# PierfrancescoArdino/C2M

Hardware: AMD Instinct MI355X
Metric: generator train-step frames/sec at 128x256x7 (higher is better)
Workload: dtype f32; 1 GPU; BASELINE configs[1]: 128x256, 7-frame clips (2 in + 5 predicted), batch 8/GPU, fp32, generator fwd+bwd only (no D), VGG loss on, random-init weights; global_batch=8, parallelism=single

## Files before the change

### c2m_amd/csrc/conv_wino4.hip

```cpp
#include "common.h"
#include "conv_types.h"
#include <stdlib.h>

struct Wino4P {
    const float* U;
    const float* X;
    float* Y;
    const float* bias;
    float* Y2;
    long y2_sn, y2_sc, y2_sh;
    int lo_y, lo_x, ext_y, ext_x;
    int M, K, nimg;
    int Hi, Wi, Ho, Wo;
    int iy0, ix0;
    int reflect;
    long in_sn, out_sn, out_sc, out_sh, out_off;
    int in_sc, in_sh;
    unsigned x_bytes;
    int nchunks, mtiles;
    int act;
    float slope;
    const float* R;
    int r_l;
};

#if !defined(W4_SKEW) && !defined(W4_FUSED)
#define W4_FUSED 1
#endif

constexpr int W4_CK = 8;
constexpr int W4_TH = 4, W4_TW = 8;
constexpr int W4_OR = 4 * W4_TH, W4_OC = 4 * W4_TW;
constexpr int W4_PH = W4_OR + 2, W4_PW = W4_OC + 2;
constexpr int W4_PITCH = 40;
constexpr int W4_PPOS = W4_PH * W4_PITCH;
constexpr int W4_ROWS = (W4_PPOS + 63) / 64;
constexpr int W4_PCS = 722;
constexpr int W4_PBUF = W4_CK * W4_PCS + 48;
constexpr int W4_TAB = W4_ROWS * 64;
constexpr int W4_VBUF = 36 * W4_CK * 32;

#define W4_BT(o0, o1, o2, o3, o4, o5, x0, x1, x2, x3, x4, x5) \
    do {                                                      \
        const float a_ = (x4) - 2.25f * (x2), b_ = 0.75f * (x3) - 1.6875f * (x1);          \
        const float c_ = (x4) - 0.5625f * (x2), e_ = 1.5f * (x3) - 0.84375f * (x1);        \
        o0 = 1.265625f * (x0) - 2.8125f * (x2) + (x4);        \
        o1 = a_ + b_; o2 = a_ - b_; o3 = c_ + e_; o4 = c_ - e_; \
        o5 = 1.265625f * (x1) - 2.8125f * (x3) + (x5);        \
    } while (0)

#ifdef W4_TRACE
__device__ unsigned long long w4_trace_buf[8 * 16 * 4 + 8 * 2];
#define W4_STAMP(i) do { if (blockIdx.x == 0 && lane == 0 && n < 16) sTr[(wave * 16 + n) * 4 + (i)] = clock64(); } while (0)
C2M_API int c2m_wino4_trace_read(unsigned long long* host) {
    return (int)hipMemcpyFromSymbol(host, HIP_SYMBOL(w4_trace_buf), sizeof(w4_trace_buf));
}
#else
#define W4_STAMP(i) do { } while (0)
#endif

__global__ __launch_bounds__(512, 2) void conv_wino4_kernel(const Wino4P p) {
    __shared__ __attribute__((aligned(16))) float smem[3 * W4_PBUF + W4_TAB + 2 * W4_VBUF];
#ifdef W4_TRACE
    __shared__ unsigned long long sTr[8 * 16 * 4 + 8 * 2];
    const unsigned long long t_begin = clock64();
#endif
#define sP (smem)
#define sVo (reinterpret_cast<unsigned*>(smem + 3 * W4_PBUF))
#define sV (smem + 3 * W4_PBUF + W4_TAB)
    const int tid = threadIdx.x, lane = tid & 63;
    const int wave = __builtin_amdgcn_readfirstlane(tid >> 6);
    const int wm = wave & 1, fg = wave >> 1;
    const bool t_first = (wave ^ (wave >> 2)) & 1;
    const int regions_x = (p.Wo + W4_OC - 1) / W4_OC, regions_y = (p.Ho + W4_OR - 1) / W4_OR;
    int rb, mt;
    {
        const unsigned L = blockIdx.x, total = gridDim.x;
        const unsigned q = total >> 3, r = total & 7u, x = L & 7u, j = L >> 3;
        const unsigned w = x * q + (x < r ? x : r) + j;
        mt = (int)(w % (unsigned)p.mtiles); rb = (int)(w / (unsigned)p.mtiles);
    }
    const int rx = rb % regions_x; rb /= regions_x;
    const int ry = rb % regions_y; const int img = rb / regions_y;
    const int oy0 = ry * W4_OR, ox0 = rx * W4_OC;
    const int nchunks = p.nchunks;

    {
        const unsigned img_byte = (unsigned)(img * (int)p.in_sn) * 4u;
        for (int pos = tid; pos < W4_TAB; pos += 512) {
            const int r = pos / W4_PITCH, c = pos % W4_PITCH;
            int iy = oy0 + p.iy0 + r, ix = ox0 + p.ix0 + c;
            if (p.reflect) {
                iy = iy < 0 ? -iy : iy; iy = iy >= p.Hi ? 2 * p.Hi - 2 - iy : iy;
                ix = ix < 0 ? -ix : ix; ix = ix >= p.Wi ? 2 * p.Wi - 2 - ix : ix;
            }
            const bool ok = pos < W4_PPOS && c < W4_PW && (unsigned)iy < (unsigned)p.Hi && (unsigned)ix < (unsigned)p.Wi;
            sVo[pos] = ok ? img_byte + (unsigned)(iy * p.in_sh + ix) * 4u : C2M_OOB;
        }
    }
    __syncthreads();

    const unsigned long xaddr = (unsigned long)p.X;
    const u32x4 rs = {(unsigned)xaddr, (unsigned)(xaddr >> 32) & 0xffffu, p.x_bytes, 0x00020000u};
    const unsigned sp_lds = (unsigned)(unsigned long)(__attribute__((address_space(3))) float*)&smem[0];
    unsigned pvo[W4_ROWS];
#pragma unroll
    for (int dr = 0; dr < W4_ROWS; ++dr) pvo[dr] = sVo[dr * 64 + lane];
    auto load_patch = [&](int chunk, int buf, const int dr0 = 0, const int dr1 = W4_ROWS) __attribute__((always_inline)) {
#ifdef W4_ZERO_RECORDS
        const int ch = chunk * W4_CK + wave;
        u32x4 rsk = rs;
        rsk[2] = (chunk < nchunks && ch < p.K) ? p.x_bytes : 0u;
#else
        int ch = chunk * W4_CK + wave;
        ch = ch < p.K ? ch : p.K - 1;
        const u32x4 rsk = rs;
#endif
        const int soff = ch * p.in_sc * 4;
#pragma unroll
        for (int dr = dr0; dr < dr1; ++dr) {
            const unsigned vo = pvo[dr];
            const unsigned dst = sp_lds + (unsigned)((buf * W4_PBUF + wave * W4_PCS + dr * 64) * 4);
            if (dr * 64 + 64 <= W4_PPOS || dr * 64 + lane < W4_PPOS)
                asm volatile("s_mov_b32 m0, %0\n\ts_nop 0\n\tbuffer_load_dword %1, %2, %3 offen lds"
                             :: "s"(dst), "v"(vo), "s"(rsk), "s"(soff) : "memory");
        }
    };
    const unsigned long uaddr = (unsigned long)p.U;
    const u32x4 urs = {(unsigned)uaddr, (unsigned)(uaddr >> 32) & 0xffffu, 0xffffffffu, 0x00020000u};
    const unsigned uvo = (unsigned)((((mt * 8 + wave) * 9) * 64 + lane) * 16);
    const unsigned ustride_b = (unsigned)p.mtiles * 8u * 9u * 64u * 16u;
    f32x4 ua[9];
    auto load_u = [&](int chunk) __attribute__((always_inline)) {
        const int s0 = (int)((unsigned)(chunk < nchunks ? chunk : 0) * ustride_b), s1 = s0 + 4096, s2 = s0 + 8192;
#pragma unroll
        for (int f = 0; f < 9; ++f)
            asm volatile("buffer_load_dwordx4 %0, %1, %2, %3 offen offset:%4"
                         : "=&v"(ua[f]) : "v"(uvo), "s"(urs), "s"(f < 4 ? s0 : (f < 8 ? s1 : s2)), "n"((f & 3) * 1024) : "memory");
    };

    f32x16 acc[9];
#pragma unroll
    for (int f = 0; f < 9; ++f)
#pragma unroll
        for (int r = 0; r < 16; ++r) acc[f][r] = 0.f;

    const int item = tid & 255, th = __builtin_amdgcn_readfirstlane(tid >> 8);
    const int tk = item >> 5, tn = item & 31;
    const int pbase = tk * W4_PCS + (4 * (tn >> 3)) * W4_PITCH + 4 * (tn & 7);
    auto transform = [&](int pb, int vb) __attribute__((always_inline)) {
        const float* __restrict__ src = sP + pb * W4_PBUF + pbase;
        float t[3][6];
#pragma unroll
        for (int cp = 0; cp < 3; ++cp) {
            f32x2 d[6];
#pragma unroll
            for (int r = 0; r < 6; ++r) d[r] = *reinterpret_cast<const f32x2*>(src + r * W4_PITCH + 2 * cp);
#pragma unroll
            for (int e = 0; e < 2; ++e) {
                const float d0 = d[0][e], d1 = d[1][e], d2 = d[2][e], d3 = d[3][e], d4 = d[4][e], d5 = d[5][e];
                const int c = 2 * cp + e;
                if (th == 0) {
                    const float a_ = d4 - 2.25f * d2, b_ = 0.75f * d3 - 1.6875f * d1;
                    t[0][c] = 1.265625f * d0 - 2.8125f * d2 + d4; t[1][c] = a_ + b_; t[2][c] = a_ - b_;
                } else {
                    const float c_ = d4 - 0.5625f * d2, e_ = 1.5f * d3 - 0.84375f * d1;
                    t[0][c] = c_ + e_; t[1][c] = c_ - e_; t[2][c] = 1.265625f * d1 - 2.8125f * d3 + d5;
                }
            }
        }
        float* __restrict__ v = sV + vb * W4_VBUF + tk * 32 + tn;
#pragma unroll
        for (int a = 0; a < 3; ++a) {
            float o0, o1, o2, o3, o4, o5;
            W4_BT(o0, o1, o2, o3, o4, o5, t[a][0], t[a][1], t[a][2], t[a][3], t[a][4], t[a][5]);
            const int xi0 = 6 * (3 * th + a);
            v[(xi0 + 0) * W4_CK * 32] = o0; v[(xi0 + 1) * W4_CK * 32] = o1; v[(xi0 + 2) * W4_CK * 32] = o2;
            v[(xi0 + 3) * W4_CK * 32] = o3; v[(xi0 + 4) * W4_CK * 32] = o4; v[(xi0 + 5) * W4_CK * 32] = o5;
            __builtin_amdgcn_sched_barrier(0);
        }
    };
    auto mma = [&](int cur, int next_chunk) __attribute__((always_inline)) {
        const float* __restrict__ vb = sV + cur * W4_VBUF + (9 * fg * W4_CK + (lane >> 5)) * 32 + (lane & 31);
        const int s0 = (int)((unsigned)(next_chunk < nchunks ? next_chunk : 0) * ustride_b), s1 = s0 + 4096, s2 = s0 + 8192;
#pragma unroll
        for (int g3 = 0; g3 < 3; ++g3) {
            float b[3][4];
#pragma unroll
            for (int f = 0; f < 3; ++f)
#pragma unroll
                for (int kk = 0; kk < 4; ++kk) b[f][kk] = vb[((3 * g3 + f) * W4_CK + 2 * kk) * 32];
#pragma unroll
            for (int kk = 0; kk < 4; ++kk)
#pragma unroll
                for (int f = 0; f < 3; ++f) {
                    const f32x4 u = ua[3 * g3 + f];
                    const float av = kk == 0 ? u.x : (kk == 1 ? u.y : (kk == 2 ? u.z : u.w));
                    acc[3 * g3 + f] = __builtin_amdgcn_mfma_f32_32x32x2f32(av, b[f][kk], acc[3 * g3 + f], 0, 0, 0);
                }
            __builtin_amdgcn_sched_barrier(0);
#pragma unroll
            for (int f = 3 * g3; f < 3 * g3 + 3; ++f)
                asm volatile("buffer_load_dwordx4 %0, %1, %2, %3 offen offset:%4"
                             : "=&v"(ua[f]) : "v"(uvo), "s"(urs), "s"(f < 4 ? s0 : (f < 8 ? s1 : s2)), "n"((f & 3) * 1024) : "memory");
            __builtin_amdgcn_sched_barrier(0);
        }
    };

#ifdef W4_FUSED
    const float cA = th ? 0.5625f : 2.25f, cB3 = th ? 1.5f : 0.75f, cB1 = th ? 0.84375f : 1.6875f;
    const int xrow = th ? 5 : 0, r_single = th ? 5 : 0, r_plus = th ? 3 : 1, r_minus = th ? 4 : 2;
    auto fused = [&](int cur, int next_chunk, int pb, int dbuf) __attribute__((always_inline)) {
        const float* __restrict__ vb = sV + cur * W4_VBUF + (9 * fg * W4_CK + (lane >> 5)) * 32 + (lane & 31);
        const float* __restrict__ src = sP + pb * W4_PBUF + pbase;
        const int s0 = (int)((unsigned)(next_chunk < nchunks ? next_chunk : 0) * ustride_b), s1 = s0 + 4096, s2 = s0 + 8192;
        float ts[6], tp[6], tm[6];
        float b[3][4];
        f32x2 d1, d2, d3, d4, dx;
        auto reads = [&](const int g3) __attribute__((always_inline)) {
#pragma unroll
            for (int f = 0; f < 3; ++f)
#pragma unroll
                for (int kk = 0; kk < 4; ++kk) b[f][kk] = vb[((3 * g3 + f) * W4_CK + 2 * kk) * 32];
            d1 = *reinterpret_cast<const f32x2*>(src + 1 * W4_PITCH + 2 * g3); d2 = *reinterpret_cast<const f32x2*>(src + 2 * W4_PITCH + 2 * g3);
            d3 = *reinterpret_cast<const f32x2*>(src + 3 * W4_PITCH + 2 * g3); d4 = *reinterpret_cast<const f32x2*>(src + 4 * W4_PITCH + 2 * g3);
            dx = *reinterpret_cast<const f32x2*>(src + xrow * W4_PITCH + 2 * g3);
        };
        asm volatile("s_waitcnt vmcnt(12)" ::: "memory");
#pragma unroll
        for (int f = 0; f < 3; ++f) asm volatile("" : "+v"(ua[f]));
        reads(0);
#pragma unroll
        for (int g3 = 0; g3 < 3; ++g3) {
#pragma unroll
            for (int kk = 0; kk < 4; ++kk)
#pragma unroll
                for (int f = 0; f < 3; ++f) {
                    const f32x4 u = ua[3 * g3 + f];
                    const float av = kk == 0 ? u.x : (kk == 1 ? u.y : (kk == 2 ? u.z : u.w));
                    acc[3 * g3 + f] = __builtin_amdgcn_mfma_f32_32x32x2f32(av, b[f][kk], acc[3 * g3 + f], 0, 0, 0);
                }
#pragma unroll
            for (int e = 0; e < 2; ++e) {
                const int c = 2 * g3 + e;
                const float q0 = th ? d1[e] : dx[e], q2 = th ? d3[e] : d2[e], q4 = th ? dx[e] : d4[e];
                ts[c] = 1.265625f * q0 - 2.8125f * q2 + q4;
                const float a_ = d4[e] - cA * d2[e], b_ = cB3 * d3[e] - cB1 * d1[e];
                tp[c] = a_ + b_; tm[c] = a_ - b_;
            }
            if (g3 == 0) __builtin_amdgcn_sched_group_barrier(0x100, 17, 0);
#pragma unroll
            for (int q = 0; q < 12; ++q) {
                __builtin_amdgcn_sched_group_barrier(0x008, 1, 0);
                __builtin_amdgcn_sched_group_barrier(0x002, 2, 0);
            }
            __builtin_amdgcn_sched_barrier(0);
            if (g3 < 2) reads(g3 + 1);
            if (g3 < 2) load_patch(next_chunk + 1, dbuf, 6 * g3, 6 * g3 + 6);
#pragma unroll
            for (int f = 3 * g3; f < 3 * g3 + 3; ++f)
                asm volatile("buffer_load_dwordx4 %0, %1, %2, %3 offen offset:%4"
                             : "=&v"(ua[f]) : "v"(uvo), "s"(urs), "s"(f < 4 ? s0 : (f < 8 ? s1 : s2)), "n"((f & 3) * 1024) : "memory");
            if (g3 == 0) asm volatile("s_waitcnt vmcnt(12)" ::: "memory");
            if (g3 == 1) asm volatile("s_waitcnt vmcnt(18)" ::: "memory");
            if (g3 < 2) {
#pragma unroll
                for (int f = 3 * g3 + 3; f < 3 * g3 + 6; ++f) asm volatile("" : "+v"(ua[f]));
            }
            __builtin_amdgcn_sched_barrier(0);
        }
        float* __restrict__ v = sV + (cur ^ 1) * W4_VBUF + tk * 32 + tn;
#pragma unroll
        for (int a = 0; a < 3; ++a) {
            const float* t = a == 0 ? ts : (a == 1 ? tp : tm);
            const int row = a == 0 ? r_single : (a == 1 ? r_plus : r_minus);
            float o0, o1, o2, o3, o4, o5;
            W4_BT(o0, o1, o2, o3, o4, o5, t[0], t[1], t[2], t[3], t[4], t[5]);
            float* __restrict__ vr = v + 6 * row * W4_CK * 32;
            vr[0] = o0; vr[1 * W4_CK * 32] = o1; vr[2 * W4_CK * 32] = o2;
            vr[3 * W4_CK * 32] = o3; vr[4 * W4_CK * 32] = o4; vr[5 * W4_CK * 32] = o5;
        }
    };
#endif

    load_patch(0, 0);
    load_patch(1, 1);
    load_u(0);
    asm volatile("s_waitcnt vmcnt(21)" ::: "memory");
    __syncthreads();
    transform(0, 0);
#ifdef W4_FUSED
    asm volatile("s_waitcnt vmcnt(0)" ::: "memory");
#else
    asm volatile("s_waitcnt vmcnt(9)" ::: "memory");
#endif
    int pn = 1;
#ifdef W4_PRIO
    if (wave >= 4) __builtin_amdgcn_s_setprio(1);
#endif
    for (int n = 0; n < nchunks; ++n) {
        __syncthreads();
        W4_STAMP(0);
        const int cur = n & 1;
        const int dbuf = pn == 2 ? 0 : pn + 1;
#ifndef W4_FUSED
        load_patch(n + 2, dbuf);
#endif
        __builtin_amdgcn_sched_barrier(0);
#ifdef W4_FUSED
        W4_STAMP(1);
        fused(cur, n + 1, pn, dbuf);
        W4_STAMP(2);
        W4_STAMP(3);
#else
        if (t_first) transform(pn, cur ^ 1);
        asm volatile("s_waitcnt vmcnt(12)" ::: "memory");
#pragma unroll
        for (int f = 0; f < 9; ++f) asm volatile("" : "+v"(ua[f]));
        W4_STAMP(1);
        mma(cur, n + 1);
        W4_STAMP(2);
        if (!t_first) transform(pn, cur ^ 1);
        W4_STAMP(3);
#endif
#ifdef W4_FUSED
        asm volatile("s_waitcnt vmcnt(6)" ::: "memory");
#else
        asm volatile("s_waitcnt vmcnt(9)" ::: "memory");
#endif
        pn = pn == 2 ? 0 : pn + 1;
    }
    asm volatile("s_waitcnt vmcnt(0)" ::: "memory");
#pragma unroll
    for (int f = 0; f < 9; ++f) asm volatile("" :: "v"(ua[f]));
    __syncthreads();

    float* __restrict__ sR = sV;
    const int etile = tid & 31, ecl = tid >> 5;
    const int ety = etile >> 3, etx = etile & 7;
    const int oyb = oy0 + 4 * ety, oxb = ox0 + 4 * etx;
    float bias4[4];
#pragma unroll
    for (int pass = 0; pass < 4; ++pass) {
        const int co = mt * 64 + (pass >> 1) * 32 + (pass & 1) * 16 + ecl;
        bias4[pass] = (p.bias && co < p.M) ? p.bias[co] : 0.f;
    }
#pragma unroll
    for (int pass = 0; pass < 4; ++pass) {
        const int pwm = pass >> 1, hf = pass & 1;
        __syncthreads();
        if (wm == pwm) {
#pragma unroll
            for (int f = 0; f < 9; ++f)
#pragma unroll
                for (int rr = 0; rr < 8; ++rr) {
                    const int rowl = (rr & 3) + 8 * (rr >> 2) + 4 * (lane >> 5);
                    sR[((9 * fg + f) * 16 + rowl) * 32 + (lane & 31)] = hf ? acc[f][8 + rr] : acc[f][rr];
                }
        }
        __syncthreads();
        const int cout = mt * 64 + pwm * 32 + hf * 16 + ecl;
        float y[4][4];
        {
            float s[6][4];
#pragma unroll
            for (int i = 0; i < 6; ++i) {
                const float* __restrict__ q = sR + ((6 * i) * 16 + ecl) * 32 + etile;
                const float m0 = q[0], m1 = q[16 * 32], m2 = q[2 * 16 * 32], m3 = q[3 * 16 * 32], m4 = q[4 * 16 * 32], m5 = q[5 * 16 * 32];
                const float pp = m1 + m2, nn = m1 - m2, PP = m3 + m4, NN = m3 - m4;
                s[i][0] = m0 + pp + PP; s[i][1] = 0.75f * nn + 1.5f * NN; s[i][2] = 0.5625f * pp + 2.25f * PP;
                s[i][3] = 0.421875f * nn + 3.375f * NN + m5;
            }
#pragma unroll
            for (int c = 0; c < 4; ++c) {
                const float pp = s[1][c] + s[2][c], nn = s[1][c] - s[2][c], PP = s[3][c] + s[4][c], NN = s[3][c] - s[4][c];
                y[0][c] = s[0][c] + pp + PP; y[1][c] = 0.75f * nn + 1.5f * NN; y[2][c] = 0.5625f * pp + 2.25f * PP;
                y[3][c] = 0.421875f * nn + 3.375f * NN + s[5][c];
            }
        }
        if (cout < p.M) {
            const float bb = bias4[pass];
            const float* __restrict__ rb = p.R ? p.R + ((long)img * p.M + cout) * 4 * p.r_l : nullptr;
#pragma unroll
            for (int r = 0; r < 4; ++r) {
                const int oy = oyb + r;
                if (oy >= p.Ho) continue;
                if (rb) {
                    if (oy == 1 || oy == p.Ho - 2) {
                        const float* __restrict__ rr = rb + (oy == 1 ? 0 : p.r_l) + oxb;
#pragma unroll
                        for (int c = 0; c < 4; ++c) if (oxb + c < p.Wo) y[r][c] += rr[c];
                    }
                    if (oxb <= 1 && oxb + 3 >= 1) {
                        const float v = rb[2 * p.r_l + oy];
#pragma unroll
                        for (int c = 0; c < 4; ++c) if (oxb + c == 1) y[r][c] += v;
                    }
                    if (oxb <= p.Wo - 2 && oxb + 3 >= p.Wo - 2) {
                        const float v = rb[3 * p.r_l + oy];
#pragma unroll
                        for (int c = 0; c < 4; ++c) if (oxb + c == p.Wo - 2) y[r][c] += v;
                    }
                }
                if (p.act == C2M_ACT_NONE) {
#pragma unroll
                    for (int c = 0; c < 4; ++c) y[r][c] += bb;
                } else if (p.act == C2M_ACT_LRELU) {
#pragma unroll
                    for (int c = 0; c < 4; ++c) { const float v = y[r][c] + bb; y[r][c] = v > 0.f ? v : p.slope * v; }
                } else {
#pragma unroll
                    for (int c = 0; c < 4; ++c) y[r][c] = c2m_act(y[r][c] + bb, p.act, p.slope);
                }
                float* __restrict__ yb0 = p.Y + p.out_off + (long)img * p.out_sn + (long)cout * p.out_sc + (long)oy * p.out_sh + oxb;
                typedef float f32x4u __attribute__((ext_vector_type(4), aligned(4)));
                const f32x4u vv = {y[r][0], y[r][1], y[r][2], y[r][3]};
                const int yi = oy - p.lo_y, xi0 = oxb - p.lo_x;
                const bool row_in = p.Y2 && (unsigned)yi < (unsigned)p.ext_y;
                const bool all_in = row_in && xi0 >= 0 && xi0 + 3 < p.ext_x;
                const bool all_out = !row_in || xi0 + 3 < 0 || xi0 >= p.ext_x;
                if (oxb + 3 < p.Wo && (!p.Y2 || all_out)) {
                    *reinterpret_cast<f32x4u*>(yb0) = vv;
                } else if (oxb + 3 < p.Wo && all_in) {
                    *reinterpret_cast<f32x4u*>(p.Y2 + (long)img * p.y2_sn + (long)cout * p.y2_sc + (long)yi * p.y2_sh + xi0) = vv;
                } else {
#pragma unroll
                    for (int c = 0; c < 4; ++c) {
                        if (oxb + c >= p.Wo) continue;
                        const int xi = oxb + c - p.lo_x;
                        if (row_in && (unsigned)xi < (unsigned)p.ext_x)
                            p.Y2[(long)img * p.y2_sn + (long)cout * p.y2_sc + (long)yi * p.y2_sh + xi] = y[r][c];
                        else
                            yb0[c] = y[r][c];
                    }
                }
            }
        }
    }
#ifdef W4_TRACE
    if (blockIdx.x == 0 && lane == 0) { sTr[8 * 16 * 4 + wave * 2] = t_begin; sTr[8 * 16 * 4 + wave * 2 + 1] = clock64(); }
    __syncthreads();
    if (blockIdx.x == 0)
        for (int i = tid; i < 8 * 16 * 4 + 8 * 2; i += 512) w4_trace_buf[i] = sTr[i];
#endif
}

#undef sP
#undef sVo
#undef sV

__global__ void wino4_filter_kernel(const float* __restrict__ w, float* __restrict__ up, int M, int K, int Cin_native,
                                    int dgrad, int mtiles, long pairs) {
    for (long i = blockIdx.x * (long)blockDim.x + threadIdx.x; i < pairs; i += (long)gridDim.x * blockDim.x) {
        const int kk = (int)(i & 3); long r = i >> 2;
        const int lane = (int)(r & 63); r >>= 6;
        const int wm = (int)(r & 1); r >>= 1;
        const int mt = (int)(r % mtiles); const int chunk = (int)(r / mtiles);
        const int m = mt * 64 + wm * 32 + (lane & 31), c = chunk * W4_CK + 2 * kk + (lane >> 5);
        float u[6][6];
#pragma unroll
        for (int a = 0; a < 6; ++a)
#pragma unroll
            for (int b2 = 0; b2 < 6; ++b2) u[a][b2] = 0.f;
        if (m < M && c < K) {
            const float* __restrict__ g = dgrad ? w + ((long)c * Cin_native + m) * 9 : w + ((long)m * Cin_native + c) * 9;
            float gg[3][3];
#pragma unroll
            for (int a = 0; a < 3; ++a)
#pragma unroll
                for (int b2 = 0; b2 < 3; ++b2) gg[a][b2] = dgrad ? g[(2 - a) * 3 + (2 - b2)] : g[a * 3 + b2];
            float row[6][3];
#pragma unroll
            for (int b2 = 0; b2 < 3; ++b2) {
                const float g0 = gg[0][b2], g1 = gg[1][b2], g2 = gg[2][b2];
                row[0][b2] = (64.f / 81.f) * g0;
                row[1][b2] = -(128.f / 243.f) * g0 - (32.f / 81.f) * g1 - (8.f / 27.f) * g2;
                row[2][b2] = -(128.f / 243.f) * g0 + (32.f / 81.f) * g1 - (8.f / 27.f) * g2;
                row[3][b2] = (32.f / 243.f) * g0 + (16.f / 81.f) * g1 + (8.f / 27.f) * g2;
                row[4][b2] = (32.f / 243.f) * g0 - (16.f / 81.f) * g1 + (8.f / 27.f) * g2;
                row[5][b2] = g2;
            }
#pragma unroll
            for (int a = 0; a < 6; ++a) {
                const float r0 = row[a][0], r1 = row[a][1], r2 = row[a][2];
                u[a][0] = (64.f / 81.f) * r0;
                u[a][1] = -(128.f / 243.f) * r0 - (32.f / 81.f) * r1 - (8.f / 27.f) * r2;
                u[a][2] = -(128.f / 243.f) * r0 + (32.f / 81.f) * r1 - (8.f / 27.f) * r2;
                u[a][3] = (32.f / 243.f) * r0 + (16.f / 81.f) * r1 + (8.f / 27.f) * r2;
                u[a][4] = (32.f / 243.f) * r0 - (16.f / 81.f) * r1 + (8.f / 27.f) * r2;
                u[a][5] = r2;
            }
        }
        const long base = ((long)chunk * mtiles + mt) * 8;
#pragma unroll
        for (int a = 0; a < 6; ++a)
#pragma unroll
            for (int b2 = 0; b2 < 6; ++b2) {
                const int xi = 6 * a + b2, fgi = xi / 9, f = xi % 9;
                up[((((base + ((fgi << 1) | wm)) * 9 + f) * 64 + lane) << 2) + kk] = u[a][b2];
            }
    }
}

C2M_API long c2m_wino4_upack_floats(int M, int K) {
    return 36L * (c2m_cdiv(M, 64) * 64L) * (c2m_cdiv(K, W4_CK) * (long)W4_CK);
}

C2M_API int c2m_wino4_filter_transform(const float* w, float* upack, int Cout, int Cin, int dgrad, void* stream) {
    C2M_ENTER();
    const int M = dgrad ? Cin : Cout, K = dgrad ? Cout : Cin;
    if (M <= 0 || K <= 0) return 0;
    const long total = c2m_wino4_upack_floats(M, K);
    if (total * 4 >= 0xffffffffL) return (int)hipErrorInvalidValue;
    hipLaunchKernelGGL(wino4_filter_kernel, dim3(c2m_grid(total / 36, 256)), dim3(256), 0, (hipStream_t)stream, w, upack, M,
                       K, Cin, dgrad, c2m_cdiv(M, 64), total / 36);
    return (int)hipGetLastError();
}

C2M_API int c2m_wino4_regions(int Ho, int Wo) { return c2m_cdiv(Ho, W4_OR) * c2m_cdiv(Wo, W4_OC); }

C2M_API int c2m_conv_wino4(const float* upack, const float* X, float* Y, float* Y_interior, const float* bias,
                           const int64_t* g, int act, float slope, void* stream) {
    C2M_ENTER();
    Wino4P p;
    p.U = upack; p.X = X; p.Y = Y; p.bias = bias;
    p.Y2 = Y_interior; p.y2_sn = p.y2_sc = p.y2_sh = 0; p.lo_y = p.lo_x = p.ext_y = p.ext_x = 0;
    if (Y_interior) {
        p.y2_sn = g[C2M_WG_Y2_SN]; p.y2_sc = g[C2M_WG_Y2_SC]; p.y2_sh = g[C2M_WG_Y2_SH];
        p.lo_y = (int)g[C2M_WG_LO_Y]; p.lo_x = (int)g[C2M_WG_LO_X]; p.ext_y = (int)g[C2M_WG_EXT_Y]; p.ext_x = (int)g[C2M_WG_EXT_X];
    }
    p.M = (int)g[C2M_WG_M]; p.K = (int)g[C2M_WG_K]; p.nimg = (int)g[C2M_WG_NIMG];
    p.Hi = (int)g[C2M_WG_HI]; p.Wi = (int)g[C2M_WG_WI]; p.Ho = (int)g[C2M_WG_HO]; p.Wo = (int)g[C2M_WG_WO];
    p.iy0 = (int)g[C2M_WG_IY0]; p.ix0 = (int)g[C2M_WG_IX0]; p.reflect = (int)g[C2M_WG_REFLECT];
    p.in_sn = g[C2M_WG_IN_SN]; p.in_sc = (int)g[C2M_WG_IN_SC]; p.in_sh = (int)g[C2M_WG_IN_SH];
    p.out_sn = g[C2M_WG_OUT_SN]; p.out_sc = g[C2M_WG_OUT_SC]; p.out_sh = g[C2M_WG_OUT_SH]; p.out_off = g[C2M_WG_OUT_OFF];
    if (g[C2M_WG_X_BYTES] <= 0 || g[C2M_WG_X_BYTES] >= 0x80000000LL) return (int)hipErrorInvalidValue;
    p.x_bytes = (unsigned)g[C2M_WG_X_BYTES];
    if (g[C2M_WG_NKT] != 0 || g[C2M_WG_PTAB] != 0) return (int)hipErrorInvalidValue;
    p.R = (const float*)(uintptr_t)g[C2M_WG_RING]; p.r_l = (int)g[C2M_WG_RING_L];
    if (p.R && (Y_interior || p.reflect || p.Ho < 4 || p.Wo < 4 || p.r_l < p.Ho || p.r_l < p.Wo || p.out_off != 0)) return (int)hipErrorInvalidValue;
    p.act = act; p.slope = slope;
    if (p.M <= 0 || p.K <= 0 || p.nimg <= 0 || p.Ho <= 0 || p.Wo <= 0) return 0;
    if ((((uintptr_t)upack) & 15) != 0) return (int)hipErrorInvalidValue;
    p.nchunks = c2m_cdiv(p.K, W4_CK);
    p.mtiles = c2m_cdiv(p.M, 64);
    if (c2m_wino4_upack_floats(p.M, p.K) * 4 >= 0xffffffffL) return (int)hipErrorInvalidValue;
    const long regions = (long)p.nimg * c2m_wino4_regions(p.Ho, p.Wo);
    if (regions * p.mtiles > 0x7fffffffL) return (int)hipErrorInvalidValue;
    hipLaunchKernelGGL(conv_wino4_kernel, dim3((unsigned)(regions * p.mtiles)), dim3(512), 0, (hipStream_t)stream, p);
    return (int)hipGetLastError();
}
```

Measured before the change: 993.9 frames/s.

## Compute gather offsets in registers and halve epilogue barrier passes in Winograd conv

Each lane now computes its patch-gather offsets directly into registers, which removes the shared-memory offset table and one block barrier. The epilogue staging is also restructured: both wm halves write their accumulators to shared memory together, so two barrier-separated passes replace four. Shared memory is reused across loop and epilogue phases. The fast path stores full 4x4 output tiles with vector stores when there is no Y2 split. The cost is more epilogue LDS per block (36*32*32 floats) and extra per-lane address math; it also adds optional trace stamps.

```diff
diff --git a/c2m_amd/csrc/conv_wino4.hip b/c2m_amd/csrc/conv_wino4.hip
--- a/c2m_amd/csrc/conv_wino4.hip
+++ b/c2m_amd/csrc/conv_wino4.hip
@@ -37,8 +37,9 @@
 constexpr int W4_ROWS = (W4_PPOS + 63) / 64;
 constexpr int W4_PCS = 722;
 constexpr int W4_PBUF = W4_CK * W4_PCS + 48;
-constexpr int W4_TAB = W4_ROWS * 64;
 constexpr int W4_VBUF = 36 * W4_CK * 32;
+constexpr int W4_LOOP = 3 * W4_PBUF + 2 * W4_VBUF;
+constexpr int W4_EPI = 36 * 32 * 32;
 
 #define W4_BT(o0, o1, o2, o3, o4, o5, x0, x1, x2, x3, x4, x5) \
     do {                                                      \
@@ -50,24 +51,27 @@
     } while (0)
 
 #ifdef W4_TRACE
-__device__ unsigned long long w4_trace_buf[8 * 16 * 4 + 8 * 2];
+constexpr int W4_TRACE_N = 8 * 16 * 4 + 8 * 2 + 8 * 16;
+__device__ unsigned long long w4_trace_buf[W4_TRACE_N];
 #define W4_STAMP(i) do { if (blockIdx.x == 0 && lane == 0 && n < 16) sTr[(wave * 16 + n) * 4 + (i)] = clock64(); } while (0)
+#define W4_PSTAMP(i) do { if (blockIdx.x == 0 && lane == 0) sTr[8 * 16 * 4 + 8 * 2 + wave * 16 + (i)] = clock64(); } while (0)
 C2M_API int c2m_wino4_trace_read(unsigned long long* host) {
     return (int)hipMemcpyFromSymbol(host, HIP_SYMBOL(w4_trace_buf), sizeof(w4_trace_buf));
 }
 #else
 #define W4_STAMP(i) do { } while (0)
+#define W4_PSTAMP(i) do { } while (0)
 #endif
 
 __global__ __launch_bounds__(512, 2) void conv_wino4_kernel(const Wino4P p) {
-    __shared__ __attribute__((aligned(16))) float smem[3 * W4_PBUF + W4_TAB + 2 * W4_VBUF];
+    __shared__ __attribute__((aligned(16))) float smem[W4_LOOP > W4_EPI ? W4_LOOP : W4_EPI];
 #ifdef W4_TRACE
-    __shared__ unsigned long long sTr[8 * 16 * 4 + 8 * 2];
+    __shared__ unsigned long long sTr[W4_TRACE_N];
     const unsigned long long t_begin = clock64();
+    if ((threadIdx.x & 63) < 16) sTr[8 * 16 * 4 + 8 * 2 + (threadIdx.x >> 6) * 16 + (threadIdx.x & 63)] = 0;
 #endif
 #define sP (smem)
-#define sVo (reinterpret_cast<unsigned*>(smem + 3 * W4_PBUF))
-#define sV (smem + 3 * W4_PBUF + W4_TAB)
+#define sV (smem + 3 * W4_PBUF)
     const int tid = threadIdx.x, lane = tid & 63;
     const int wave = __builtin_amdgcn_readfirstlane(tid >> 6);
     const int wm = wave & 1, fg = wave >> 1;
@@ -85,9 +89,12 @@
     const int oy0 = ry * W4_OR, ox0 = rx * W4_OC;
     const int nchunks = p.nchunks;
 
+    unsigned pvo[W4_ROWS];
     {
         const unsigned img_byte = (unsigned)(img * (int)p.in_sn) * 4u;
-        for (int pos = tid; pos < W4_TAB; pos += 512) {
+#pragma unroll
+        for (int dr = 0; dr < W4_ROWS; ++dr) {
+            const int pos = dr * 64 + lane;
             const int r = pos / W4_PITCH, c = pos % W4_PITCH;
             int iy = oy0 + p.iy0 + r, ix = ox0 + p.ix0 + c;
             if (p.reflect) {
@@ -95,17 +102,14 @@
                 ix = ix < 0 ? -ix : ix; ix = ix >= p.Wi ? 2 * p.Wi - 2 - ix : ix;
             }
             const bool ok = pos < W4_PPOS && c < W4_PW && (unsigned)iy < (unsigned)p.Hi && (unsigned)ix < (unsigned)p.Wi;
-            sVo[pos] = ok ? img_byte + (unsigned)(iy * p.in_sh + ix) * 4u : C2M_OOB;
-        }
-    }
-    __syncthreads();
+            pvo[dr] = ok ? img_byte + (unsigned)(iy * p.in_sh + ix) * 4u : C2M_OOB;
+        }
+    }
+    W4_PSTAMP(0);
 
     const unsigned long xaddr = (unsigned long)p.X;
     const u32x4 rs = {(unsigned)xaddr, (unsigned)(xaddr >> 32) & 0xffffu, p.x_bytes, 0x00020000u};
     const unsigned sp_lds = (unsigned)(unsigned long)(__attribute__((address_space(3))) float*)&smem[0];
-    unsigned pvo[W4_ROWS];
-#pragma unroll
-    for (int dr = 0; dr < W4_ROWS; ++dr) pvo[dr] = sVo[dr * 64 + lane];
     auto load_patch = [&](int chunk, int buf, const int dr0 = 0, const int dr1 = W4_ROWS) __attribute__((always_inline)) {
 #ifdef W4_ZERO_RECORDS
         const int ch = chunk * W4_CK + wave;
@@ -288,12 +292,15 @@
     load_u(0);
     asm volatile("s_waitcnt vmcnt(21)" ::: "memory");
     __syncthreads();
+    W4_PSTAMP(1);
     transform(0, 0);
+    W4_PSTAMP(2);
 #ifdef W4_FUSED
     asm volatile("s_waitcnt vmcnt(0)" ::: "memory");
 #else
     asm volatile("s_waitcnt vmcnt(9)" ::: "memory");
 #endif
+    W4_PSTAMP(3);
     int pn = 1;
 #ifdef W4_PRIO
     if (wave >= 4) __builtin_amdgcn_s_setprio(1);
@@ -334,9 +341,11 @@
 #pragma unroll
     for (int f = 0; f < 9; ++f) asm volatile("" :: "v"(ua[f]));
     __syncthreads();
-
-    float* __restrict__ sR = sV;
-    const int etile = tid & 31, ecl = tid >> 5;
+    W4_PSTAMP(4);
+
+    float* __restrict__ sR = smem;
+    const int elane = (int)__builtin_amdgcn_mbcnt_hi(~0u, __builtin_amdgcn_mbcnt_lo(~0u, 0u));
+    const int etile = elane & 31, ecl = 2 * wave + (elane >> 5);
     const int ety = etile >> 3, etx = etile & 7;
     const int oyb = oy0 + 4 * ety, oxb = ox0 + 4 * etx;
     float bias4[4];
@@ -346,107 +355,131 @@
         bias4[pass] = (p.bias && co < p.M) ? p.bias[co] : 0.f;
     }
 #pragma unroll
-    for (int pass = 0; pass < 4; ++pass) {
-        const int pwm = pass >> 1, hf = pass & 1;
+    for (int hf = 0; hf < 2; ++hf) {
+        if (hf) __syncthreads();
+#pragma unroll
+        for (int f = 0; f < 9; ++f)
+#pragma unroll
+            for (int rr = 0; rr < 8; ++rr) {
+                const int rowl = (rr & 3) + 8 * (rr >> 2) + 4 * (elane >> 5);
+                sR[((9 * fg + f) * 32 + wm * 16 + rowl) * 32 + etile] = hf ? acc[f][8 + rr] : acc[f][rr];
+            }
         __syncthreads();
-        if (wm == pwm) {
-#pragma unroll
-            for (int f = 0; f < 9; ++f)
-#pragma unroll
-                for (int rr = 0; rr < 8; ++rr) {
-                    const int rowl = (rr & 3) + 8 * (rr >> 2) + 4 * (lane >> 5);
-                    sR[((9 * fg + f) * 16 + rowl) * 32 + (lane & 31)] = hf ? acc[f][8 + rr] : acc[f][rr];
-                }
-        }
-        __syncthreads();
-        const int cout = mt * 64 + pwm * 32 + hf * 16 + ecl;
-        float y[4][4];
-        {
-            float s[6][4];
-#pragma unroll
-            for (int i = 0; i < 6; ++i) {
-                const float* __restrict__ q = sR + ((6 * i) * 16 + ecl) * 32 + etile;
-                const float m0 = q[0], m1 = q[16 * 32], m2 = q[2 * 16 * 32], m3 = q[3 * 16 * 32], m4 = q[4 * 16 * 32], m5 = q[5 * 16 * 32];
-                const float pp = m1 + m2, nn = m1 - m2, PP = m3 + m4, NN = m3 - m4;
-                s[i][0] = m0 + pp + PP; s[i][1] = 0.75f * nn + 1.5f * NN; s[i][2] = 0.5625f * pp + 2.25f * PP;
-                s[i][3] = 0.421875f * nn + 3.375f * NN + m5;
-            }
-#pragma unroll
-            for (int c = 0; c < 4; ++c) {
-                const float pp = s[1][c] + s[2][c], nn = s[1][c] - s[2][c], PP = s[3][c] + s[4][c], NN = s[3][c] - s[4][c];
-                y[0][c] = s[0][c] + pp + PP; y[1][c] = 0.75f * nn + 1.5f * NN; y[2][c] = 0.5625f * pp + 2.25f * PP;
-                y[3][c] = 0.421875f * nn + 3.375f * NN + s[5][c];
-            }
-        }
-        if (cout < p.M) {
-            const float bb = bias4[pass];
-            const float* __restrict__ rb = p.R ? p.R + ((long)img * p.M + cout) * 4 * p.r_l : nullptr;
-#pragma unroll
-            for (int r = 0; r < 4; ++r) {
-                const int oy = oyb + r;
-                if (oy >= p.Ho) continue;
-                if (rb) {
-                    if (oy == 1 || oy == p.Ho - 2) {
-                        const float* __restrict__ rr = rb + (oy == 1 ? 0 : p.r_l) + oxb;
-#pragma unroll
-                        for (int c = 0; c < 4; ++c) if (oxb + c < p.Wo) y[r][c] += rr[c];
+        W4_PSTAMP(5 + 2 * hf);
+#pragma unroll
+        for (int pwm = 0; pwm < 2; ++pwm) {
+            const int pass = 2 * pwm + hf;
+            const int cout = mt * 64 + pwm * 32 + hf * 16 + ecl;
+            float y[4][4];
+            {
+                float s[6][4];
+#pragma unroll
+                for (int i = 0; i < 6; ++i) {
+                    const float* __restrict__ q = sR + ((6 * i) * 32 + pwm * 16 + ecl) * 32 + etile;
+                    const float m0 = q[0], m1 = q[32 * 32], m2 = q[2 * 32 * 32], m3 = q[3 * 32 * 32], m4 = q[4 * 32 * 32], m5 = q[5 * 32 * 32];
+                    const float pp = m1 + m2, nn = m1 - m2, PP = m3 + m4, NN = m3 - m4;
+                    s[i][0] = m0 + pp + PP; s[i][1] = 0.75f * nn + 1.5f * NN; s[i][2] = 0.5625f * pp + 2.25f * PP;
+                    s[i][3] = 0.421875f * nn + 3.375f * NN + m5;
+                }
+#pragma unroll
+                for (int c = 0; c < 4; ++c) {
+                    const float pp = s[1][c] + s[2][c], nn = s[1][c] - s[2][c], PP = s[3][c] + s[4][c], NN = s[3][c] - s[4][c];
+                    y[0][c] = s[0][c] + pp + PP; y[1][c] = 0.75f * nn + 1.5f * NN; y[2][c] = 0.5625f * pp + 2.25f * PP;
+                    y[3][c] = 0.421875f * nn + 3.375f * NN + s[5][c];
+                }
+            }
+            if (pass == 3) W4_PSTAMP(14);
+            if (cout < p.M) {
+                const float bb = bias4[pass];
+                if (p.R) {
+                    const float* __restrict__ rb = p.R + ((long)img * p.M + cout) * 4 * p.r_l;
+#pragma unroll
+                    for (int r = 0; r < 4; ++r) {
+                        const int oy = oyb + r;
+                        if (oy >= p.Ho) continue;
+                        if (oy == 1 || oy == p.Ho - 2) {
+                            const float* __restrict__ rr = rb + (oy == 1 ? 0 : p.r_l) + oxb;
+#pragma unroll
+                            for (int c = 0; c < 4; ++c) if (oxb + c < p.Wo) y[r][c] += rr[c];
+                        }
+                        if (oxb <= 1 && oxb + 3 >= 1) {
+                            const float v = rb[2 * p.r_l + oy];
+#pragma unroll
+                            for (int c = 0; c < 4; ++c) if (oxb + c == 1) y[r][c] += v;
+                        }
+                        if (oxb <= p.Wo - 2 && oxb + 3 >= p.Wo - 2) {
+                            const float v = rb[3 * p.r_l + oy];
+#pragma unroll
+                            for (int c = 0; c < 4; ++c) if (oxb + c == p.Wo - 2) y[r][c] += v;
+                        }
                     }
-                    if (oxb <= 1 && oxb + 3 >= 1) {
-                        const float v = rb[2 * p.r_l + oy];
-#pragma unroll
-                        for (int c = 0; c < 4; ++c) if (oxb + c == 1) y[r][c] += v;
+                }
+                if (p.act == C2M_ACT_NONE) {
+#pragma unroll
+                    for (int r = 0; r < 4; ++r)
+#pragma unroll
+                        for (int c = 0; c < 4; ++c) y[r][c] += bb;
+                } else if (p.act == C2M_ACT_LRELU) {
+#pragma unroll
+                    for (int r = 0; r < 4; ++r)
+#pragma unroll
+                        for (int c = 0; c < 4; ++c) { const float v = y[r][c] + bb; y[r][c] = v > 0.f ? v : p.slope * v; }
+                } else {
+#pragma unroll
+                    for (int r = 0; r < 4; ++r)
+#pragma unroll
+                        for (int c = 0; c < 4; ++c) y[r][c] = c2m_act(y[r][c] + bb, p.act, p.slope);
+                }
+                typedef float f32x4u __attribute__((ext_vector_type(4), aligned(4)));
+                float* __restrict__ yb = p.Y + p.out_off + (long)img * p.out_sn + (long)cout * p.out_sc + (long)oyb * p.out_sh + oxb;
+                if (!p.Y2 && oyb + 3 < p.Ho && oxb + 3 < p.Wo) {
+#pragma unroll
+                    for (int r = 0; r < 4; ++r) {
+                        const f32x4u vv = {y[r][0], y[r][1], y[r][2], y[r][3]};
+                        *reinterpret_cast<f32x4u*>(yb + (long)r * p.out_sh) = vv;
                     }
-                    if (oxb <= p.Wo - 2 && oxb + 3 >= p.Wo - 2) {
-                        const float v = rb[3 * p.r_l + oy];
-#pragma unroll
-                        for (int c = 0; c < 4; ++c) if (oxb + c == p.Wo - 2) y[r][c] += v;
+                } else {
+#pragma unroll
+                    for (int r = 0; r < 4; ++r) {
+                        const int oy = oyb + r;
+                        if (oy >= p.Ho) continue;
+                        float* __restrict__ yb0 = yb + (long)r * p.out_sh;
+                        const f32x4u vv = {y[r][0], y[r][1], y[r][2], y[r][3]};
+                        const int yi = oy - p.lo_y, xi0 = oxb - p.lo_x;
+                        const bool row_in = p.Y2 && (unsigned)yi < (unsigned)p.ext_y;
+                        const bool all_in = row_in && xi0 >= 0 && xi0 + 3 < p.ext_x;
+                        const bool all_out = !row_in || xi0 + 3 < 0 || xi0 >= p.ext_x;
+                        if (oxb + 3 < p.Wo && (!p.Y2 || all_out)) {
+                            *reinterpret_cast<f32x4u*>(yb0) = vv;
+                        } else if (oxb + 3 < p.Wo && all_in) {
+                            *reinterpret_cast<f32x4u*>(p.Y2 + (long)img * p.y2_sn + (long)cout * p.y2_sc + (long)yi * p.y2_sh + xi0) = vv;
+                        } else {
+#pragma unroll
+                            for (int c = 0; c < 4; ++c) {
+                                if (oxb + c >= p.Wo) continue;
+                                const int xi = oxb + c - p.lo_x;
+                                if (row_in && (unsigned)xi < (unsigned)p.ext_x)
+                                    p.Y2[(long)img * p.y2_sn + (long)cout * p.y2_sc + (long)yi * p.y2_sh + xi] = y[r][c];
+                                else
+                                    yb0[c] = y[r][c];
+                            }
+                        }
                     }
                 }
-                if (p.act == C2M_ACT_NONE) {
-#pragma unroll
-                    for (int c = 0; c < 4; ++c) y[r][c] += bb;
-                } else if (p.act == C2M_ACT_LRELU) {
-#pragma unroll
-                    for (int c = 0; c < 4; ++c) { const float v = y[r][c] + bb; y[r][c] = v > 0.f ? v : p.slope * v; }
-                } else {
-#pragma unroll
-                    for (int c = 0; c < 4; ++c) y[r][c] = c2m_act(y[r][c] + bb, p.act, p.slope);
-                }
-                float* __restrict__ yb0 = p.Y + p.out_off + (long)img * p.out_sn + (long)cout * p.out_sc + (long)oy * p.out_sh + oxb;
-                typedef float f32x4u __attribute__((ext_vector_type(4), aligned(4)));
-                const f32x4u vv = {y[r][0], y[r][1], y[r][2], y[r][3]};
-                const int yi = oy - p.lo_y, xi0 = oxb - p.lo_x;
-                const bool row_in = p.Y2 && (unsigned)yi < (unsigned)p.ext_y;
-                const bool all_in = row_in && xi0 >= 0 && xi0 + 3 < p.ext_x;
-                const bool all_out = !row_in || xi0 + 3 < 0 || xi0 >= p.ext_x;
-                if (oxb + 3 < p.Wo && (!p.Y2 || all_out)) {
-                    *reinterpret_cast<f32x4u*>(yb0) = vv;
-                } else if (oxb + 3 < p.Wo && all_in) {
-                    *reinterpret_cast<f32x4u*>(p.Y2 + (long)img * p.y2_sn + (long)cout * p.y2_sc + (long)yi * p.y2_sh + xi0) = vv;
-                } else {
-#pragma unroll
-                    for (int c = 0; c < 4; ++c) {
-                        if (oxb + c >= p.Wo) continue;
-                        const int xi = oxb + c - p.lo_x;
-                        if (row_in && (unsigned)xi < (unsigned)p.ext_x)
-                            p.Y2[(long)img * p.y2_sn + (long)cout * p.y2_sc + (long)yi * p.y2_sh + xi] = y[r][c];
-                        else
-                            yb0[c] = y[r][c];
-                    }
-                }
-            }
-        }
+            }
+            if (pass == 1) W4_PSTAMP(13);
+        }
+        W4_PSTAMP(6 + 2 * hf);
     }
 #ifdef W4_TRACE
     if (blockIdx.x == 0 && lane == 0) { sTr[8 * 16 * 4 + wave * 2] = t_begin; sTr[8 * 16 * 4 + wave * 2 + 1] = clock64(); }
     __syncthreads();
     if (blockIdx.x == 0)
-        for (int i = tid; i < 8 * 16 * 4 + 8 * 2; i += 512) w4_trace_buf[i] = sTr[i];
+        for (int i = tid; i < W4_TRACE_N; i += 512) w4_trace_buf[i] = sTr[i];
 #endif
 }
 
 #undef sP
-#undef sVo
 #undef sV
 
 __global__ void wino4_filter_kernel(const float* __restrict__ w, float* __restrict__ up, int M, int K, int Cin_native,
```

After: 1009 frames/s, median of 6. +1.5%, better.
